# JuliaHealth/Thunderbolt.jl

Hardware: AMD Instinct MI355X
Metric: element-integrations/sec + DoF-updates/sec, 10M-hex Q1 monodomain (higher is better)
Workload: dtype f64

## Files before the change

### thunderbolt.jl_amd/csrc/tb_reaction.hip

```cpp
#include <hip/hip_runtime.h>

#include <cstdlib>
#include <type_traits>

#include "tb_internal.h"
#include "tb_math.hpp"

namespace tb {

struct CellParams {
    double p[48];
};

template <int MODEL> struct CellModel;

template <> struct CellModel<TB_CELL_FHN> {
    static constexpr int NS = 2, PHI = 0;
    static constexpr bool HAS_GATES = false;
    __device__ __forceinline__ static void rhs(const CellParams &P, const double (&u)[NS], double, double (&du)[NS])
    {
        const double a = P.p[0], b = P.p[1], c = P.p[2], d = P.p[3], e = P.p[4], f = P.p[5];
        const double phi = u[0], s = u[1];
        du[0] = f * (phi * (1 - phi) * (phi - a) - s);
        du[1] = e * (b * phi - c * s - d);
    }
};

template <> struct CellModel<TB_CELL_ALIEV_PANFILOV> {
    static constexpr int NS = 2, PHI = 1;
    static constexpr bool HAS_GATES = false;
    __device__ __forceinline__ static void rhs(const CellParams &P, const double (&u)[NS], double, double (&du)[NS])
    {
        const double ct = P.p[0], k = P.p[1], a = P.p[2], e0 = P.p[3], mu1 = P.p[4], mu2 = P.p[5];
        const double phi = u[1], s = u[0];
        const double eps = e0 + s * mu1 / (phi + mu2);
        du[1] = ct * (k * phi * (phi - 1.0) * (phi - a) - phi * s);
        du[0] = ct * eps * (-s - k * phi * (phi - a - 1.0));
    }
};

template <> struct CellModel<TB_CELL_PCG2019> {
    static constexpr int NS = 7, PHI = 0;
    static constexpr bool HAS_GATES = true;
    enum { gNa, Em, km, taum, Eh, kh, dh, tauh0, gK1, Ez, kz, gto, Er, kr, Es, ks, taus, gCaL, Ed, kd, Ef, kf, tauf,
           gKr, Exr, kxr, tauxr, Ey, ky, gKs, Exs, kxs, tauxs, ENa, EK, ECa };
    __device__ __forceinline__ static double sigmoid(double phi, double E, double ik, double sign)
    {
        return rcp_b(1.0 + exp_b(sign * (phi - E) * ik));
    }
    __device__ __forceinline__ static void rhs(const CellParams &P, const double (&u)[NS], double t, double (&du)[NS])
    {
        double rate[NS];
        rhs_rates(P, u, t, du, rate);
    }
    __device__ __forceinline__ static void rhs_rates(const CellParams &P, const double (&u)[NS], double, double (&du)[NS], double (&rate)[NS])
    {
        const double *p = P.p;
        const double phi = u[0], h = u[1], m = u[2], f = u[3], s = u[4], xs = u[5], xr = u[6];
        const double rinf = sigmoid(phi, p[Er], 1.0 / p[kr], -1.0);
        const double dinf = sigmoid(phi, p[Ed], 1.0 / p[kd], -1.0);
        const double zinf = sigmoid(phi, p[Ez], 1.0 / p[kz], 1.0);
        const double yinf = sigmoid(phi, p[Ey], 1.0 / p[ky], 1.0);
        const double I_Na = p[gNa] * m * m * m * h * h * (phi - p[ENa]);
        const double I_K1 = p[gK1] * zinf * (phi - p[EK]);
        const double I_to = p[gto] * rinf * s * (phi - p[EK]);
        const double I_CaL = p[gCaL] * dinf * f * (phi - p[ECa]);
        const double I_Kr = p[gKr] * xr * yinf * (phi - p[EK]);
        const double I_Ks = p[gKs] * xs * (phi - p[EK]);
        du[0] = -(I_Na + I_K1 + I_to + I_CaL + I_Kr + I_Ks);
        const double xh = (phi - p[Eh]) * (1.0 / p[kh]);
        const double eh = exp_b(xh);
        const double hinf = rcp_b(1.0 + eh);
        rate[0] = 0.0; rate[1] = (1.0 + eh) * exp_b(-p[dh] * xh) * (0.5 / p[tauh0]); rate[2] = 1.0 / p[taum]; rate[3] = 1.0 / p[tauf]; rate[4] = 1.0 / p[taus];
        rate[5] = 1.0 / p[tauxs]; rate[6] = 1.0 / p[tauxr];
        du[1] = (hinf - h) * rate[1];
        du[2] = (sigmoid(phi, p[Em], 1.0 / p[km], -1.0) - m) * rate[2];
        du[3] = (sigmoid(phi, p[Ef], 1.0 / p[kf], 1.0) - f) * rate[3];
        du[4] = (sigmoid(phi, p[Es], 1.0 / p[ks], 1.0) - s) * rate[4];
        du[5] = (sigmoid(phi, p[Exs], 1.0 / p[kxs], -1.0) - xs) * rate[5];
        du[6] = (sigmoid(phi, p[Exr], 1.0 / p[kxr], -1.0) - xr) * rate[6];
    }
};

template <> struct CellModel<TB_CELL_FHN_HETEROGENEOUS> {
    static constexpr int NS = 2, PHI = 0;
    static constexpr bool HAS_GATES = false, USES_X = true;
    __device__ __forceinline__ static void rhs_x(const CellParams &P, const double (&u)[NS], const float (&x)[3], double, double (&du)[NS])
    {
        const double a = P.p[0], b = P.p[1], c = P.p[2], d = P.p[3];
        const double e = P.p[4] + P.p[5] * (double)x[0] + P.p[6] * (double)x[1] + P.p[7] * (double)x[2];
        const double phi = u[0], s = u[1];
        du[0] = phi * (1.0 - phi) * (phi - a) - s;
        du[1] = e * (b * phi - c * s - d);
    }
};


template <> struct CellModel<TB_CELL_TT06> {
    static constexpr int NS = 19, PHI = 0;
    __device__ __forceinline__ static double sgm(double e) { return rcp_b(1.0 + e); }
    static constexpr bool HAS_GATES = true;
    __device__ __forceinline__ static void rhs(const CellParams &P, const double (&u)[NS], double t, double (&du)[NS])
    {
        double rate[NS];
        rhs_rates(P, u, t, du, rate);
    }
    __device__ __forceinline__ static void rhs_rates(const CellParams &P, const double (&u)[NS], double, double (&du)[NS], double (&rate)[NS])
    {
#pragma unroll
        for (int k = 0; k < NS; ++k) rate[k] = 0.0;
        const double *p = P.p;
        const double GNa = p[0], GK1 = p[1], GKr = p[2], GKs = p[3], Gto = p[4], GCaL = p[5], GbNa = p[6], GbCa = p[7], GpCa = p[8],
                     GpK = p[9], knak = p[10], knaca = p[11], Ko = p[12], Cao = p[13], Nao = p[14], Vc = p[15], Vsr = p[16], Vss = p[17],
                     Bufc = p[18], Kbufc = p[19], Bufsr = p[20], Kbufsr = p[21], Bufss = p[22], Kbufss = p[23], Vmaxup = p[24], Kup = p[25],
                     Vrel = p[26], k1p = p[27], k2p = p[28], k3 = p[29], k4 = p[30], EC = p[31], maxsr = p[32], minsr = p[33],
                     Vleak = p[34], Vxfer = p[35], Cm = p[36], pKNa = p[37], KmK = p[38], KmNa = p[39], KmNai = p[40], KmCa = p[41],
                     ksat = p[42], nn = p[43], KpCa = p[44], R = p[45], T = p[46], F = p[47];
        const double V = u[0], Cai = u[1], CaSR = u[2], CaSS = u[3], Nai = u[4], Ki = u[5], m = u[6], h = u[7], j = u[8], xr1 = u[9],
                     xr2 = u[10], xs = u[11], r = u[12], s = u[13], d = u[14], f = u[15], f2 = u[16], fCass = u[17], RR = u[18];
        const double RTONF = R * T / F, FoRT = F / (R * T);
        const double Ek = RTONF * (log(Ko) - log_b(Ki)), Ena = RTONF * (log(Nao) - log_b(Nai));
        const double Eks = RTONF * (log(Ko + pKNa * Nao) - log_b(Ki + pKNa * Nai)), Eca = 0.5 * RTONF * (log(Cao) - log_b(Cai));
        const double p5 = exp_b(V * (1.0 / 5.0)), q5 = rcp_b(p5);
        const double p10 = exp_b(V * (1.0 / 10.0)), q10 = rcp_b(p10);
        const double p20 = exp_b(V * (1.0 / 20.0)), q20 = rcp_b(p20);
        const double p7 = exp_b(V * (1.0 / 7.0)), q7 = rcp_b(p7);
        const double q6 = exp_b(-V * (1.0 / 6.0));
        const double w = exp_b(V * FoRT), iw = rcp_b(w);
        const double vk = V - Ek;
        const double Ak1 = 0.1 * sgm(exp_b(0.06 * (vk - 200.0)));
        const double eh = exp_b(-0.5 * vk);
        const double Bk1 = (3.0 * exp_b(0.0002 * (vk + 100.0)) + exp_b(0.1 * (vk - 10.0))) * sgm(eh);
        const double INa = GNa * m * m * m * h * j * (V - Ena);
        const double e2 = w * w * exp_b(-30.0 * FoRT);
        const double ICaL = GCaL * d * f * f2 * fCass * 4.0 * (V - 15.0) * (F * FoRT) * (0.25 * e2 * CaSS - Cao) * rcp_b(e2 - 1.0);
        const double Ito = Gto * r * s * vk;
        const double IKr = GKr * sqrt(Ko * (1.0 / 5.4)) * xr1 * xr2 * vk;
        const double IKs = GKs * xs * xs * (V - Eks);
        const double IK1 = GK1 * (Ak1 * rcp_b(Ak1 + Bk1)) * vk;
        const double en = exp_b(nn * V * FoRT), en1 = en * iw;
        const double INaCa = knaca * (1.0 / (KmNai * KmNai * KmNai + Nao * Nao * Nao)) * (1.0 / (KmCa + Cao)) * rcp_b(1.0 + ksat * en1) *
                             (en * Nai * Nai * Nai * Cao - en1 * Nao * Nao * Nao * Cai * 2.5);
        const double INaK = knak * (Ko / (Ko + KmK)) * (Nai * rcp_b(Nai + KmNa)) * rcp_b(1.0 + 0.1245 * exp_b(-0.1 * V * FoRT) + 0.0353 * iw);
        const double IpCa = GpCa * Cai * rcp_b(KpCa + Cai);
        const double IpK = GpK * sgm(exp_b((25.0 - V) * (1.0 / 5.98))) * vk;
        const double IbNa = GbNa * (V - Ena), IbCa = GbCa * (V - Eca);
        du[0] = -(IKr + IKs + IK1 + Ito + INa + IbNa + ICaL + IbCa + INaK + INaCa + IpCa + IpK);
        const double ecs = EC * rcp_b(CaSR);
        const double kCaSR = maxsr - (maxsr - minsr) * rcp_b(1.0 + ecs * ecs);
        const double k1 = k1p * rcp_b(kCaSR), k2 = k2p * kCaSR;
        du[18] = k4 * (1.0 - RR) - k2 * CaSS * RR;
        const double O = k1 * CaSS * CaSS * RR * rcp_b(k3 + k1 * CaSS * CaSS);
        const double Irel = Vrel * O * (CaSR - CaSS), Ileak = Vleak * (CaSR - Cai);
        const double Iup = Vmaxup * (Cai * Cai) * rcp_b(Cai * Cai + Kup * Kup), Ixfer = Vxfer * (CaSS - Cai);
        const double sc = (Cai + Kbufc) * (Cai + Kbufc), ssr = (CaSR + Kbufsr) * (CaSR + Kbufsr), sss = (CaSS + Kbufss) * (CaSS + Kbufss);
        const double bc = sc * rcp_b(sc + Bufc * Kbufc), bsr = ssr * rcp_b(ssr + Bufsr * Kbufsr), bss = sss * rcp_b(sss + Bufss * Kbufss);
        du[1] = bc * ((Ileak - Iup) * Vsr / Vc + Ixfer - (IbCa + IpCa - 2.0 * INaCa) * Cm / (2.0 * Vc * F));
        du[2] = bsr * (Iup - Irel - Ileak);
        du[3] = bss * (-ICaL * Cm / (2.0 * Vss * F) + Irel * Vsr / Vss - Ixfer * Vc / Vss);
        du[4] = -(INa + IbNa + 3.0 * INaK + 3.0 * INaCa) * Cm / (Vc * F);
        du[5] = -(IK1 + Ito + IKr + IKs - 2.0 * INaK + IpK) * Cm / (Vc * F);
        const double AM = sgm(q5 * 6.14421235332821e-06 );
        const double BM = 0.1 * sgm(p5 * 1096.6331584284585 ) + 0.1 * sgm(exp_b((V - 50.0) * (1.0 / 200.0)));
        const double mr = sgm(exp_b((-56.86 - V) * (1.0 / 9.03)));
        rate[6] = rcp_b(AM * BM);
        du[6] = (mr * mr - m) * rate[6];
        const double hr = sgm(exp_b((V + 71.55) * (1.0 / 7.43)));
        const double hinf = hr * hr;
        double ABH, ABJ;
        if (V >= -40.0) {
            ABH = (0.77 / 0.13) * sgm(exp_b(-(V + 10.66) * (1.0 / 11.1)));
            ABJ = 0.6 * exp_b(0.057 * V) * sgm(q10 * 0.04076220397836621 );
        } else {
            ABH = 0.057 * exp_b(-(V + 80.0) * (1.0 / 6.8)) + 2.7 * exp_b(0.079 * V) + 3.1e5 * exp_b(0.3485 * V);
            ABJ = ((-2.5428e4) * exp_b(0.2444 * V) - 6.948e-6 * exp_b(-0.04391 * V)) * (V + 37.78) * sgm(exp_b(0.311 * (V + 79.23))) +
                  0.02424 * exp_b(-0.01052 * V) * sgm(exp_b(-0.1378 * (V + 40.14)));
        }
        rate[7] = ABH;
        du[7] = (hinf - h) * ABH;
        rate[8] = ABJ;
        du[8] = (hinf - j) * ABJ;
        rate[9] = rcp_b((450.0 * sgm(q10 * 0.011108996538242306 )) * (6.0 * sgm(exp_b((V + 30.0) * (1.0 / 11.5)))));
        du[9] = (sgm(q7 * 0.02437284407327961 ) - xr1) * rate[9];
        rate[10] = rcp_b((3.0 * sgm(q20 * 0.049787068367863944 )) * (1.12 * sgm(p20 * 0.049787068367863944 )));
        du[10] = (sgm(exp_b((V + 88.0) * (1.0 / 24.0))) - xr2) * rate[10];
        rate[11] = rcp_b((1400.0 / sqrt(1.0 + q6 * 2.3009758908928246 )) * sgm(exp_b((V - 35.0) * (1.0 / 15.0))) + 80.0);
        du[11] = (sgm(exp_b((-5.0 - V) * (1.0 / 14.0))) - xs) * rate[11];
        rate[12] = rcp_b(9.5 * exp_b(-(V + 40.0) * (V + 40.0) * (1.0 / 1800.0)) + 0.8);
        du[12] = (sgm(q6 * 28.031624894526125 ) - r) * rate[12];
        rate[13] = rcp_b(85.0 * exp_b(-(V + 45.0) * (V + 45.0) * (1.0 / 320.0)) + 5.0 * sgm(p5 * 0.01831563888873418 ) + 3.0);
        du[13] = (sgm(p5 * 54.598150033144236 ) - s) * rate[13];
        rate[14] = rcp_b((1.4 * sgm(exp_b((-35.0 - V) * (1.0 / 13.0))) + 0.25) * (1.4 * sgm(p5 * 2.718281828459045 )) + sgm(q20 * 12.182493960703473 ));
        du[14] = (sgm(exp_b((-8.0 - V) * (1.0 / 7.5))) - d) * rate[14];
        rate[15] = rcp_b((1102.5 * exp_b(-(V + 27.0) * (V + 27.0) * (1.0 / 225.0)) + 200.0 * sgm(q10 * 3.6692966676192444 ) + 180.0 * sgm(p10 * 20.085536923187668 ) + 20.0));
        du[15] = (sgm(p7 * 17.411708063327644 ) - f) * rate[15];
        rate[16] = rcp_b((600.0 * exp_b(-(V + 25.0) * (V + 25.0) * (1.0 / 170.0)) + 31.0 * sgm(q10 * 12.182493960703473 ) + 16.0 * sgm(p10 * 20.085536923187668 )));
        du[16] = (0.67 * sgm(p7 * 148.4131591025766 ) + 0.33 - f2) * rate[16];
        const double cq = 1.0 + (CaSS * (1.0 / 0.05)) * (CaSS * (1.0 / 0.05));
        const double icq = rcp_b(cq);
        rate[17] = rcp_b(80.0 * icq + 2.0);
        du[17] = (0.6 * icq + 0.4 - fCass) * rate[17];
    }
};


template <> struct CellModel<TB_CELL_ORD11> {
    static constexpr int NS = 41, PHI = 0;
    static constexpr bool HAS_GATES = true;
    __device__ __forceinline__ static double sg(double x) { return rcp_b(1.0 + exp_b(x)); }
    __device__ __forceinline__ static void rhs(const CellParams &P, const double (&u)[NS], double t, double (&du)[NS])
    {
        double rate[NS];
        rhs_rates(P, u, t, du, rate);
    }
    __device__ __forceinline__ static void currents(const CellParams &P, const double (&u)[NS], double (&du)[NS])
    {
        const double *p = P.p;
        const double nao = p[13], cao = p[14], ko = p[15];
        const int celltype = (int)p[16];
        constexpr double R = 8314.0, T = 310.0, F = 96485.0, RTF = R * T / F, FRT = F / (R * T);
        constexpr double L = 0.01, rad = 0.0011, vcell = 1000 * 3.14 * rad * rad * L, Ageo = 2 * 3.14 * rad * rad + 2 * 3.14 * rad * L, Acap = 2 * Ageo;
        constexpr double vmyo = 0.68 * vcell, vnsr = 0.0552 * vcell, vjsr = 0.0048 * vcell, vss = 0.02 * vcell;
        const double v = u[0], nai = u[1], nass = u[2], ki = u[3], kss = u[4], cai = u[5], cass = u[6], cansr = u[7], cajsr = u[8], m = u[9], hf = u[10],
                     hs = u[11], j = u[12], hsp = u[13], jp = u[14], mL = u[15], hL = u[16], hLp = u[17], a = u[18], iF = u[19], iS = u[20],
                     ap = u[21], iFp = u[22], iSp = u[23], d = u[24], ff = u[25], fs = u[26], fcaf = u[27], fcas = u[28], jca = u[29], nca = u[30],
                     ffp = u[31], fcafp = u[32], xrf = u[33], xrs = u[34], xs1 = u[35], xs2 = u[36], xk1 = u[37], Jrelnp = u[38], Jrelp = u[39],
                     CaMKt = u[40];
        constexpr double KmCaMK = 0.15, aCaMK = 0.05, bCaMK = 0.00068, CaMKo = 0.05, KmCaM = 0.0015;
        const double CaMKb = CaMKo * (1.0 - CaMKt) * cass * rcp_b(cass + KmCaM), CaMKa = CaMKb + CaMKt;
        du[40] = aCaMK * CaMKb * (CaMKb + CaMKt) - bCaMK * CaMKt;
        const double fpa = CaMKa * rcp_b(CaMKa + KmCaMK), fnp = 1.0 - fpa;
        const double ENa = RTF * (log(nao) - log(nai)), EK = RTF * (log(ko) - log(ki));
        const double EKs = RTF * (log(ko + 0.01833 * nao) - log(ki + 0.01833 * nai));
        const double vg = fabs(v) < 1e-7 ? 1e-7 : v;
        const double vfrt = vg * FRT, vffrt = vfrt * F;
        constexpr double Ahf = 0.99, Ahs = 1.0 - Ahf;
        const double h = Ahf * hf + Ahs * hs;
        const double hp = Ahf * hf + Ahs * hsp;
        const double INa = 75.0 * p[0] * (v - ENa) * m * m * m * (fnp * h * j + fpa * hp * jp);
        const double INaL = 0.0075 * p[1] * (celltype == 1 ? 0.6 : 1.0) * (v - ENa) * mL * (fnp * hL + fpa * hLp);
        const double AiF = sg((v - 213.6) * (1.0 / 151.2)), AiS = 1.0 - AiF;
        const double i_ = AiF * iF + AiS * iS;
        const double ip = AiF * iFp + AiS * iSp;
        const double Ito = 0.02 * p[2] * (celltype == 0 ? 1.0 : 4.0) * (v - EK) * (fnp * a * i_ + fpa * ap * ip);
        constexpr double Aff = 0.6, Afs = 1.0 - Aff;
        const double f = Aff * ff + Afs * fs;
        const double Afcaf = 0.3 + 0.6 * sg((v - 10.0) * (1.0 / 10.0)), Afcas = 1.0 - Afcaf;
        const double fca = Afcaf * fcaf + Afcas * fcas;
        const double fp = Aff * ffp + Afs * fs;
        const double fcap = Afcaf * fcafp + Afcas * fcas;
        constexpr double Kmn = 0.002, k2n = 1000.0;
        const double km2n = jca;
        const double q1 = 1.0 + Kmn * rcp_b(cass), q2 = q1 * q1;
        const double anca = rcp_b(k2n * rcp_b(km2n) + q2 * q2);
// ... 105 lines not shown
        const double hssp = sg((v + 89.1) * (1.0 / 6.086));
        const double mLss = sg(-(v + 42.85) * (1.0 / 5.264));
        const double hLss = sg((v + 87.61) * (1.0 / 7.488)), hLssp = sg((v + 93.81) * (1.0 / 7.488));
        const double ass = sg(-(v - 14.34) * (1.0 / 14.82));
        const double ta = 1.0515 * rcp_b(sg(-(v - 18.4099) * (1.0 / 29.3814)) * (1.0 / 1.2089) + 3.5 * sg((v + 100.0) * (1.0 / 29.3814)));
        const double iss = sg((v + 43.94) * (1.0 / 5.711));
        const double delta_epi = celltype == 1 ? 1.0 - 0.95 * sg((v + 70.0) * (1.0 / 5.0)) : 1.0;
        const double tiF = (4.562 + rcp_b(0.3933 * exp_b(-(v + 100.0) * (1.0 / 100.0)) + 0.08004 * exp_b((v + 50.0) * (1.0 / 16.59)))) * delta_epi;
        const double tiS = (23.62 + rcp_b(0.001416 * exp_b(-(v + 96.52) * (1.0 / 59.05)) + 1.780e-8 * exp_b((v + 114.1) * (1.0 / 8.079)))) * delta_epi;
        const double assp = sg(-(v - 24.34) * (1.0 / 14.82));
        const double dti_develop = 1.354 + 1.0e-4 * rcp_b(exp_b((v - 167.4) * (1.0 / 15.89)) + exp_b(-(v - 12.23) * (1.0 / 0.2154)));
        const double dti_recover = 1.0 - 0.5 * sg((v + 70.0) * (1.0 / 20.0));
        const double tiFp = dti_develop * dti_recover * tiF, tiSp = dti_develop * dti_recover * tiS;
        const double dss = sg(-(v + 3.940) * (1.0 / 4.230));
        const double td = 0.6 + rcp_b(exp_b(-0.05 * (v + 6.0)) + exp_b(0.09 * (v + 14.0)));
        const double fss = sg((v + 19.58) * (1.0 / 3.696));
        const double e20 = exp_b((v + 20.0) * (1.0 / 10.0));
        const double tff = 7.0 + rcp_b(0.0045 * rcp_b(e20) + 0.0045 * e20);
        const double tfs = 1000.0 + rcp_b(0.000035 * exp_b(-(v + 5.0) * (1.0 / 4.0)) + 0.000035 * exp_b((v + 5.0) * (1.0 / 6.0)));
        const double e4 = exp_b((v - 4.0) * (1.0 / 7.0));
        const double tfcaf = 7.0 + rcp_b(0.04 * rcp_b(e4) + 0.04 * e4);
        const double tfcas = 100.0 + rcp_b(0.00012 * exp_b(-v * (1.0 / 3.0)) + 0.00012 * exp_b(v * (1.0 / 7.0)));
        const double xrss = sg(-(v + 8.337) * (1.0 / 6.789));
        const double txrf = 12.98 + rcp_b(0.3652 * exp_b((v - 31.66) * (1.0 / 3.869)) + 4.123e-5 * exp_b(-(v - 47.78) * (1.0 / 20.38)));
        const double txrs = 1.865 + rcp_b(0.06629 * exp_b((v - 34.70) * (1.0 / 7.355)) + 1.128e-5 * exp_b(-(v - 29.74) * (1.0 / 25.94)));
        const double xs1ss = sg(-(v + 11.60) * (1.0 / 8.932));
        const double txs1 = 817.3 + rcp_b(2.326e-4 * exp_b((v + 48.28) * (1.0 / 17.80)) + 0.001292 * exp_b(-(v + 210.0) * (1.0 / 230.0)));
        const double txs2_r = 0.01 * exp_b((v - 50.0) * (1.0 / 20.0)) + 0.0193 * exp_b(-(v + 66.54) * (1.0 / 31.0));
        const double xk1ss = sg(-(v + 2.5538 * ko + 144.59) / (1.5692 * ko + 3.8115));
        const double txk1_r = (exp_b(-(v + 127.2) * (1.0 / 20.36)) + exp_b((v + 236.8) * (1.0 / 69.33))) * (1.0 / 122.2);
        emit(9, mss, tm_r); emit(10, hss, thf_r); emit(11, hss, ths_r);
        const double rtj = rcp_b(tj);
        emit(12, hss, rtj); emit(13, hssp, ths_r * (1.0 / 3.0)); emit(14, hss, rtj * (1.0 / 1.46));
        emit(15, mLss, tm_r); emit(16, hLss, 1.0 / 200.0); emit(17, hLssp, 1.0 / 600.0);
        const double rta = rcp_b(ta);
        emit(18, ass, rta); emit(19, iss, rcp_b(tiF)); emit(20, iss, rcp_b(tiS)); emit(21, assp, rta); emit(22, iss, rcp_b(tiFp)); emit(23, iss, rcp_b(tiSp));
        emit(24, dss, rcp_b(td)); emit(25, fss, rcp_b(tff)); emit(26, fss, rcp_b(tfs)); emit(27, fss, rcp_b(tfcaf)); emit(28, fss, rcp_b(tfcas));
        emit(29, fss, 1.0 / 75.0); emit(31, fss, rcp_b(tff) * (1.0 / 2.5)); emit(32, fss, rcp_b(tfcaf) * (1.0 / 2.5));
        emit(33, xrss, rcp_b(txrf)); emit(34, xrss, rcp_b(txrs)); emit(35, xs1ss, rcp_b(txs1)); emit(36, xs1ss, txs2_r); emit(37, xk1ss, txk1_r);
    }
    __device__ __forceinline__ static bool is_gate(int k) { return (k >= 9 && k <= 29) || (k >= 31 && k <= 37); }
    __device__ __forceinline__ static void rhs_rates(const CellParams &P, const double (&u)[NS], double, double (&du)[NS], double (&rate)[NS])
    {
#pragma unroll
        for (int k = 0; k < NS; ++k) rate[k] = 0.0;
        currents(P, u, du);
        gates(P, u[0], [&](int k, double inf, double r) { rate[k] = r; du[k] = (inf - u[k]) * r; });
    }
};

template <class M, class = void> struct uses_x : std::false_type {};
template <class M> struct uses_x<M, std::enable_if_t<M::USES_X>> : std::true_type {};

template <class M>
__device__ __forceinline__ void cell_rhs(const CellParams &P, const double (&u)[M::NS], const float (&x)[3], double t, double (&du)[M::NS])
{
    if constexpr (uses_x<M>::value) M::rhs_x(P, u, x, t, du);
    else M::rhs(P, u, t, du);
}

template <int MODEL, int LAYOUT, bool WRITE_DU, class TS = double>
__global__ void __launch_bounds__(256)
k_reaction(CellParams P, TS *__restrict__ u, TS *__restrict__ du_out, int64_t n, double t, double dt, int substeps,
           double threshold, unsigned long long *__restrict__ rmax_key, const float *__restrict__ xs, int sdim, const double *__restrict__ tslot)
{
    if (tslot) t = tslot[0];
    using M = CellModel<MODEL>;
    constexpr int NS = M::NS;
    const int64_t stride = (int64_t)gridDim.x * blockDim.x;
    double rm = -__builtin_huge_val();
    for (int64_t i = (int64_t)blockIdx.x * blockDim.x + threadIdx.x; i < n; i += stride) {
        double ul[NS], dul[NS];
#pragma unroll
        for (int j = 0; j < NS; ++j) ul[j] = LAYOUT == TB_LAYOUT_SOA ? u[i + j * n] : u[i * NS + j];
        float xp[3] = {0.0f, 0.0f, 0.0f};
        if constexpr (uses_x<M>::value) {
            if (xs) for (int d = 0; d < sdim; ++d) xp[d] = xs[i * sdim + d];
        }
        cell_rhs<M>(P, ul, xp, t, dul);
        if (substeps <= 1 || fabs(dul[M::PHI]) < threshold) {
#pragma unroll
            for (int j = 0; j < NS; ++j) ul[j] += dt * dul[j];
        } else {
            const double dts = dt / substeps;
#pragma unroll
            for (int j = 0; j < NS; ++j) ul[j] += dts * dul[j];
            for (int s = 2; s <= substeps; ++s) {
                cell_rhs<M>(P, ul, xp, t + (s - 1) * dts, dul);
#pragma unroll
                for (int j = 0; j < NS; ++j) ul[j] += dts * dul[j];
            }
        }
#pragma unroll
        for (int j = 0; j < NS; ++j) {
            const int64_t k = LAYOUT == TB_LAYOUT_SOA ? i + j * n : i * NS + j;
            u[k] = (TS)ul[j];
            if (WRITE_DU) du_out[k] = (TS)dul[j];
        }
        rm = fmax(rm, dul[M::PHI]);
    }
    if (rmax_key) {
#pragma unroll
        for (int o = 32; o > 0; o >>= 1) rm = fmax(rm, __shfl_xor(rm, o, 64));
        if ((threadIdx.x & 63) == 0) {
            const unsigned long long b = (unsigned long long)__double_as_longlong(rm);
            atomicMax(rmax_key, (b >> 63) ? ~b : (b | 0x8000000000000000ull));
        }
    }
}

__device__ __forceinline__ double expm1_b(double z)
{
    if (fabs(z) < 0.3) {
        double q = 1.6059043836821613e-10;
        const double c[11] = {2.08767569878681e-09, 2.505210838544172e-08, 2.755731922398589e-07, 2.7557319223985893e-06, 2.48015873015873e-05,
                              0.0001984126984126984, 0.001388888888888889, 0.008333333333333333, 0.041666666666666664, 0.16666666666666666, 0.5};
#pragma unroll
        for (int i = 0; i < 11; ++i) q = fma(q, z, c[i]);
        q = fma(q, z, 1.0);
        return q * z;
    }
    return exp_b(z) - 1.0;
}

template <int MODEL, int LAYOUT>
__global__ void __launch_bounds__(256)
k_reaction_rl(CellParams P, double *__restrict__ u, int64_t n, double t, double dt, const double *__restrict__ tslot)
{
    if (tslot) t = tslot[0];
    using M = CellModel<MODEL>;
    constexpr int NS = M::NS;
    const int64_t stride = (int64_t)gridDim.x * blockDim.x;
    for (int64_t i = (int64_t)blockIdx.x * blockDim.x + threadIdx.x; i < n; i += stride) {
        double ul[NS], dul[NS], rate[NS];
#pragma unroll
        for (int j = 0; j < NS; ++j) ul[j] = LAYOUT == TB_LAYOUT_SOA ? u[i + j * n] : u[i * NS + j];
        M::rhs_rates(P, ul, t, dul, rate);
#pragma unroll
        for (int j = 0; j < NS; ++j) {
            const double h = rate[j] != 0.0 ? -expm1_b(-dt * rate[j]) * rcp_b(rate[j]) : dt;
            const int64_t k = LAYOUT == TB_LAYOUT_SOA ? i + j * n : i * NS + j;
            u[k] = ul[j] + h * dul[j];
        }
    }
}

int launch_reaction_rl(tb_device *dev, int model, const double *params, int n_params, double *d_u, int64_t n, int layout, double t, double dt)
{
    if (model != TB_CELL_TT06 && model != TB_CELL_PCG2019 && model != TB_CELL_ORD11) {
        set_error("Rush–Larsen step: cell model %d has no gate decomposition (TB_CELL_TT06, TB_CELL_PCG2019 and TB_CELL_ORD11 have)", model);
        return TB_ERR_UNSUPPORTED;
    }
    CellParams P{};
    for (int i = 0; i < n_params && i < 48; ++i) P.p[i] = params[i];
    int64_t nb = (n + 255) / 256;
    const int64_t cap = (int64_t)dev->n_cu * 16;
    if (nb > cap) nb = (nb + (nb + cap - 1) / cap - 1) / ((nb + cap - 1) / cap);
    if (n == 0) return TB_OK;
    const double *ts = dev->capturing ? (dev->tslot_used = true, dev->d_tslot) : nullptr;
#define TB_RL(MODEL) do { if (layout == TB_LAYOUT_SOA) hipLaunchKernelGGL((k_reaction_rl<MODEL, TB_LAYOUT_SOA>), dim3((unsigned)nb), dim3(256), 0, dev->stream, P, d_u, n, t, dt, ts); \
                          else hipLaunchKernelGGL((k_reaction_rl<MODEL, TB_LAYOUT_AOS>), dim3((unsigned)nb), dim3(256), 0, dev->stream, P, d_u, n, t, dt, ts); } while (0)
    if (model == TB_CELL_TT06) TB_RL(TB_CELL_TT06); else if (model == TB_CELL_ORD11) TB_RL(TB_CELL_ORD11); else TB_RL(TB_CELL_PCG2019);
#undef TB_RL
    TB_HIP(hipGetLastError());
    return TB_OK;
}

template <int MODEL, class TS = double>
static int run(tb_device *dev, const CellParams &P, TS *u, TS *du, int64_t n, int layout, double t, double dt, int substeps,
               double thr, unsigned long long *rmax_key, const float *xs, int sdim)
{
    const int bs = 256;
    auto launch = [&](auto kern) -> int {
        static struct { const void *f; int occ; } seen[8];
        int occ = 0;
        for (auto &e : seen) if (e.f == (const void *)kern) occ = e.occ;
        if (!occ) {
            if (hipOccupancyMaxActiveBlocksPerMultiprocessor(&occ, kern, bs, 0) != hipSuccess || occ < 1) occ = 1;
            for (auto &e : seen) if (!e.f) { e.f = (const void *)kern; e.occ = occ; break; }
        }
        int64_t nb = (n + bs - 1) / bs;
        static const int per_cu_env = tune_env("TB_REACTION_BLOCKS_PER_CU") ? atoi(tune_env("TB_REACTION_BLOCKS_PER_CU")) : -1;
        const int64_t resident = (int64_t)dev->n_cu * occ;
        const int64_t cap = per_cu_env > 0 ? (int64_t)dev->n_cu * per_cu_env : per_cu_env == 0 ? nb : (nb <= 12 * resident ? resident : 2 * resident);
        if (nb > cap) nb = (nb + (nb + cap - 1) / cap - 1) / ((nb + cap - 1) / cap);
        hipLaunchKernelGGL(kern, dim3((unsigned)nb), dim3(bs), 0, dev->stream, P, u, du, n, t, dt, substeps, thr, rmax_key, xs, sdim,
                           dev->capturing ? (dev->tslot_used = true, (const double *)dev->d_tslot) : (const double *)nullptr);
        return TB_OK;
    };
    if (layout == TB_LAYOUT_SOA) { if (du) launch(k_reaction<MODEL, TB_LAYOUT_SOA, true, TS>); else launch(k_reaction<MODEL, TB_LAYOUT_SOA, false, TS>); }
    else { if (du) launch(k_reaction<MODEL, TB_LAYOUT_AOS, true, TS>); else launch(k_reaction<MODEL, TB_LAYOUT_AOS, false, TS>); }
    TB_HIP(hipGetLastError());
    return TB_OK;
}

int launch_reaction_f32(tb_device *dev, int model, const double *params, int n_params, float *d_u, float *d_du, int64_t n_points,
                        int layout, double t, double dt, int substeps, double thr, const float *d_x, int sdim)
{
    CellParams P{};
    for (int i = 0; i < n_params && i < 48; ++i) P.p[i] = params[i];
    switch (model) {
    case TB_CELL_FHN: return run<TB_CELL_FHN, float>(dev, P, d_u, d_du, n_points, layout, t, dt, substeps, thr, nullptr, d_x, sdim);
    case TB_CELL_ALIEV_PANFILOV: return run<TB_CELL_ALIEV_PANFILOV, float>(dev, P, d_u, d_du, n_points, layout, t, dt, substeps, thr, nullptr, d_x, sdim);
    case TB_CELL_PCG2019: return run<TB_CELL_PCG2019, float>(dev, P, d_u, d_du, n_points, layout, t, dt, substeps, thr, nullptr, d_x, sdim);
    case TB_CELL_TT06: return run<TB_CELL_TT06, float>(dev, P, d_u, d_du, n_points, layout, t, dt, substeps, thr, nullptr, d_x, sdim);
    case TB_CELL_FHN_HETEROGENEOUS: return run<TB_CELL_FHN_HETEROGENEOUS, float>(dev, P, d_u, d_du, n_points, layout, t, dt, substeps, thr, nullptr, d_x, sdim);
    case TB_CELL_ORD11: return run<TB_CELL_ORD11, float>(dev, P, d_u, d_du, n_points, layout, t, dt, substeps, thr, nullptr, d_x, sdim);
    default: set_error("unknown cell model %d", model); return TB_ERR_BAD_ARG;
    }
}

int launch_reaction(tb_device *dev, int model, const double *params, int n_params, double *d_u, double *d_du, int64_t n_points,
                    int layout, double t, double dt, int substeps, double thr, double *rmax, const float *d_x, int sdim)
{
    CellParams P{};
    for (int i = 0; i < n_params && i < 48; ++i) P.p[i] = params[i];
    unsigned long long *key = nullptr;
    if (rmax) {
        TB_NO_CAPTURE(dev);
        key = (unsigned long long *)&dev->d_status->cell;
        TB_HIP(hipMemsetAsync(key, 0, sizeof *key, dev->stream));
    }
    int rc = TB_ERR_BAD_ARG;
    switch (model) {
    case TB_CELL_FHN: rc = run<TB_CELL_FHN>(dev, P, d_u, d_du, n_points, layout, t, dt, substeps, thr, key, d_x, sdim); break;
// ... 17 lines not shown
```

Before: 11.38 billion.

## Fold TT06 constants on host and algebraically simplify gate rate expressions

Precomputes the TT06 parameter-only subexpressions (log of external concentrations, volume ratios, NaCa and NaK prefactors and similar) on the host into a folded parameter struct passed to the kernel. The per-cell math is rewritten to share exponentials (p5 and p10 derived from p20 by squaring) and to merge nested reciprocals of sigmoids into single divisions, cutting transcendental and rcp counts. Loop-invariant n is also hidden behind an opaque inline asm so that strided SoA address computation stays scalar. The rewritten expressions can differ slightly in rounding from the original formulas.

Result: faster. 11.54 billion, median of 6 (+1.4%).

```diff
diff --git a/thunderbolt.jl_amd/csrc/tb_reaction.hip b/thunderbolt.jl_amd/csrc/tb_reaction.hip
--- a/thunderbolt.jl_amd/csrc/tb_reaction.hip
+++ b/thunderbolt.jl_amd/csrc/tb_reaction.hip
@@ -1,5 +1,6 @@
 #include <hip/hip_runtime.h>
 
+#include <cmath>
 #include <cstdlib>
 #include <type_traits>
 
@@ -96,19 +97,22 @@
 };
 
 
+struct TT06Folded {
+    enum { GNa, GK1, GKr , GKs, Gto, GCaL , GbNa, GbCa, GpCa, GpK, NaK , KmNa,
+           NaCa1 , NaCa2 , ksat, Cao, KpCa,
+           RTONF, Ek0 , Ena0 , Eks0 , Eca0 , pKNa, FoRT,
+           E30 , nnFoRT, EC2 , maxsr, dsr , k1p, k2p, k3, k4, Vrel, Vleak, Vmaxup, Kup2, Vxfer,
+           Kbufc, BKc , Kbufsr, BKsr, Kbufss, BKss, VsrVc , CaVc , CaVss ,
+           VsrVss, VcVss, NaVc , NF };
+    double c[NF];
+    __host__ __device__ double operator[](int k) const { return c[k]; }
+};
+
 template <> struct CellModel<TB_CELL_TT06> {
     static constexpr int NS = 19, PHI = 0;
-    __device__ __forceinline__ static double sgm(double e) { return rcp_b(1.0 + e); }
-    static constexpr bool HAS_GATES = true;
-    __device__ __forceinline__ static void rhs(const CellParams &P, const double (&u)[NS], double t, double (&du)[NS])
-    {
-        double rate[NS];
-        rhs_rates(P, u, t, du, rate);
-    }
-    __device__ __forceinline__ static void rhs_rates(const CellParams &P, const double (&u)[NS], double, double (&du)[NS], double (&rate)[NS])
-    {
-#pragma unroll
-        for (int k = 0; k < NS; ++k) rate[k] = 0.0;
+    using Params = TT06Folded;
+    static TT06Folded fold(const CellParams &P)
+    {
         const double *p = P.p;
         const double GNa = p[0], GK1 = p[1], GKr = p[2], GKs = p[3], Gto = p[4], GCaL = p[5], GbNa = p[6], GbCa = p[7], GpCa = p[8],
                      GpK = p[9], knak = p[10], knaca = p[11], Ko = p[12], Cao = p[13], Nao = p[14], Vc = p[15], Vsr = p[16], Vss = p[17],
@@ -116,54 +120,88 @@
                      Vrel = p[26], k1p = p[27], k2p = p[28], k3 = p[29], k4 = p[30], EC = p[31], maxsr = p[32], minsr = p[33],
                      Vleak = p[34], Vxfer = p[35], Cm = p[36], pKNa = p[37], KmK = p[38], KmNa = p[39], KmNai = p[40], KmCa = p[41],
                      ksat = p[42], nn = p[43], KpCa = p[44], R = p[45], T = p[46], F = p[47];
+        const double RTONF = R * T / F, FoRT = F / (R * T);
+        const double naca = knaca * (1.0 / (KmNai * KmNai * KmNai + Nao * Nao * Nao)) * (1.0 / (KmCa + Cao));
+        TT06Folded f{};
+        double *c = f.c;
+        c[TT06Folded::GNa] = GNa; c[TT06Folded::GK1] = GK1; c[TT06Folded::GKr] = GKr * std::sqrt(Ko * (1.0 / 5.4)); c[TT06Folded::GKs] = GKs;
+        c[TT06Folded::Gto] = Gto; c[TT06Folded::GCaL] = GCaL * 4.0 * (F * FoRT); c[TT06Folded::GbNa] = GbNa; c[TT06Folded::GbCa] = GbCa;
+        c[TT06Folded::GpCa] = GpCa; c[TT06Folded::GpK] = GpK; c[TT06Folded::NaK] = knak * (Ko / (Ko + KmK)); c[TT06Folded::KmNa] = KmNa;
+        c[TT06Folded::NaCa1] = naca * Cao; c[TT06Folded::NaCa2] = naca * (Nao * Nao * Nao * 2.5); c[TT06Folded::ksat] = ksat;
+        c[TT06Folded::Cao] = Cao; c[TT06Folded::KpCa] = KpCa;
+        c[TT06Folded::RTONF] = RTONF; c[TT06Folded::Ek0] = RTONF * std::log(Ko); c[TT06Folded::Ena0] = RTONF * std::log(Nao);
+        c[TT06Folded::Eks0] = RTONF * std::log(Ko + pKNa * Nao); c[TT06Folded::Eca0] = 0.5 * RTONF * std::log(Cao); c[TT06Folded::pKNa] = pKNa;
+        c[TT06Folded::FoRT] = FoRT; c[TT06Folded::E30] = std::exp(-30.0 * FoRT); c[TT06Folded::nnFoRT] = nn * FoRT;
+        c[TT06Folded::EC2] = EC * EC; c[TT06Folded::maxsr] = maxsr; c[TT06Folded::dsr] = maxsr - minsr; c[TT06Folded::k1p] = k1p;
+        c[TT06Folded::k2p] = k2p; c[TT06Folded::k3] = k3; c[TT06Folded::k4] = k4; c[TT06Folded::Vrel] = Vrel; c[TT06Folded::Vleak] = Vleak;
+        c[TT06Folded::Vmaxup] = Vmaxup; c[TT06Folded::Kup2] = Kup * Kup; c[TT06Folded::Vxfer] = Vxfer;
+        c[TT06Folded::Kbufc] = Kbufc; c[TT06Folded::BKc] = Bufc * Kbufc; c[TT06Folded::Kbufsr] = Kbufsr; c[TT06Folded::BKsr] = Bufsr * Kbufsr;
+        c[TT06Folded::Kbufss] = Kbufss; c[TT06Folded::BKss] = Bufss * Kbufss;
+        c[TT06Folded::VsrVc] = Vsr / Vc; c[TT06Folded::CaVc] = Cm / (2.0 * Vc * F); c[TT06Folded::CaVss] = Cm / (2.0 * Vss * F);
+        c[TT06Folded::VsrVss] = Vsr / Vss; c[TT06Folded::VcVss] = Vc / Vss; c[TT06Folded::NaVc] = Cm / (Vc * F);
+        return f;
+    }
+    __device__ __forceinline__ static double sgm(double e) { return rcp_b(1.0 + e); }
+    static constexpr bool HAS_GATES = true;
+    __device__ __forceinline__ static void rhs(const TT06Folded &c, const double (&u)[NS], double t, double (&du)[NS])
+    {
+        double rate[NS];
+        rhs_rates(c, u, t, du, rate);
+    }
+    __device__ __forceinline__ static void rhs_rates(const TT06Folded &c, const double (&u)[NS], double, double (&du)[NS], double (&rate)[NS])
+    {
+        using C = TT06Folded;
+#pragma unroll
+        for (int k = 0; k < NS; ++k) rate[k] = 0.0;
         const double V = u[0], Cai = u[1], CaSR = u[2], CaSS = u[3], Nai = u[4], Ki = u[5], m = u[6], h = u[7], j = u[8], xr1 = u[9],
                      xr2 = u[10], xs = u[11], r = u[12], s = u[13], d = u[14], f = u[15], f2 = u[16], fCass = u[17], RR = u[18];
-        const double RTONF = R * T / F, FoRT = F / (R * T);
-        const double Ek = RTONF * (log(Ko) - log_b(Ki)), Ena = RTONF * (log(Nao) - log_b(Nai));
-        const double Eks = RTONF * (log(Ko + pKNa * Nao) - log_b(Ki + pKNa * Nai)), Eca = 0.5 * RTONF * (log(Cao) - log_b(Cai));
-        const double p5 = exp_b(V * (1.0 / 5.0)), q5 = rcp_b(p5);
-        const double p10 = exp_b(V * (1.0 / 10.0)), q10 = rcp_b(p10);
-        const double p20 = exp_b(V * (1.0 / 20.0)), q20 = rcp_b(p20);
+        const double RTONF = c[C::RTONF], FoRT = c[C::FoRT];
+        const double Ek = fma(-RTONF, log_b(Ki), c[C::Ek0]), Ena = fma(-RTONF, log_b(Nai), c[C::Ena0]);
+        const double Eks = fma(-RTONF, log_b(Ki + c[C::pKNa] * Nai), c[C::Eks0]), Eca = fma(-0.5 * RTONF, log_b(Cai), c[C::Eca0]);
+        const double p20 = exp_b(V * (1.0 / 20.0)), p10 = p20 * p20, p5 = p10 * p10;
+        const double q20 = rcp_b(p20), q10 = q20 * q20, q5 = q10 * q10;
         const double p7 = exp_b(V * (1.0 / 7.0)), q7 = rcp_b(p7);
         const double q6 = exp_b(-V * (1.0 / 6.0));
         const double w = exp_b(V * FoRT), iw = rcp_b(w);
         const double vk = V - Ek;
-        const double Ak1 = 0.1 * sgm(exp_b(0.06 * (vk - 200.0)));
-        const double eh = exp_b(-0.5 * vk);
-        const double Bk1 = (3.0 * exp_b(0.0002 * (vk + 100.0)) + exp_b(0.1 * (vk - 10.0))) * sgm(eh);
-        const double INa = GNa * m * m * m * h * j * (V - Ena);
-        const double e2 = w * w * exp_b(-30.0 * FoRT);
-        const double ICaL = GCaL * d * f * f2 * fCass * 4.0 * (V - 15.0) * (F * FoRT) * (0.25 * e2 * CaSS - Cao) * rcp_b(e2 - 1.0);
-        const double Ito = Gto * r * s * vk;
-        const double IKr = GKr * sqrt(Ko * (1.0 / 5.4)) * xr1 * xr2 * vk;
-        const double IKs = GKs * xs * xs * (V - Eks);
-        const double IK1 = GK1 * (Ak1 * rcp_b(Ak1 + Bk1)) * vk;
-        const double en = exp_b(nn * V * FoRT), en1 = en * iw;
-        const double INaCa = knaca * (1.0 / (KmNai * KmNai * KmNai + Nao * Nao * Nao)) * (1.0 / (KmCa + Cao)) * rcp_b(1.0 + ksat * en1) *
-                             (en * Nai * Nai * Nai * Cao - en1 * Nao * Nao * Nao * Cai * 2.5);
-        const double INaK = knak * (Ko / (Ko + KmK)) * (Nai * rcp_b(Nai + KmNa)) * rcp_b(1.0 + 0.1245 * exp_b(-0.1 * V * FoRT) + 0.0353 * iw);
-        const double IpCa = GpCa * Cai * rcp_b(KpCa + Cai);
-        const double IpK = GpK * sgm(exp_b((25.0 - V) * (1.0 / 5.98))) * vk;
-        const double IbNa = GbNa * (V - Ena), IbCa = GbCa * (V - Eca);
+        const double a1 = exp_b(0.06 * (vk - 200.0)), g = exp_b(0.1 * vk), g2 = g * g, g5 = g2 * g2 * g;
+        const double Bk = 3.0 * exp_b(0.0002 * (vk + 100.0)) + g * 0.36787944117144233 ;
+        const double nk1 = 0.1 * (g5 + 1.0);
+        const double xk1 = nk1 * rcp_b(fma(Bk * (1.0 + a1), g5, nk1));
+        const double INa = c[C::GNa] * m * m * m * h * j * (V - Ena);
+        const double e2 = w * w * c[C::E30];
+        const double ICaL = c[C::GCaL] * d * f * f2 * fCass * (V - 15.0) * (0.25 * e2 * CaSS - c[C::Cao]) * rcp_b(e2 - 1.0);
+        const double Ito = c[C::Gto] * r * s * vk;
+        const double IKr = c[C::GKr] * xr1 * xr2 * vk;
+        const double IKs = c[C::GKs] * xs * xs * (V - Eks);
+        const double IK1 = c[C::GK1] * xk1 * vk;
+        const double en = exp_b(c[C::nnFoRT] * V), en1 = en * iw;
+        const double INaCa = rcp_b(fma(c[C::ksat], en1, 1.0)) * (en * Nai * Nai * Nai * c[C::NaCa1] - en1 * Cai * c[C::NaCa2]);
+        const double INaK = c[C::NaK] * Nai * rcp_b((Nai + c[C::KmNa]) * (1.0 + 0.1245 * exp_b(-0.1 * V * FoRT) + 0.0353 * iw));
+        const double IpCa = c[C::GpCa] * Cai * rcp_b(c[C::KpCa] + Cai);
+        const double IpK = c[C::GpK] * sgm(exp_b((25.0 - V) * (1.0 / 5.98))) * vk;
+        const double IbNa = c[C::GbNa] * (V - Ena), IbCa = c[C::GbCa] * (V - Eca);
         du[0] = -(IKr + IKs + IK1 + Ito + INa + IbNa + ICaL + IbCa + INaK + INaCa + IpCa + IpK);
-        const double ecs = EC * rcp_b(CaSR);
-        const double kCaSR = maxsr - (maxsr - minsr) * rcp_b(1.0 + ecs * ecs);
-        const double k1 = k1p * rcp_b(kCaSR), k2 = k2p * kCaSR;
-        du[18] = k4 * (1.0 - RR) - k2 * CaSS * RR;
-        const double O = k1 * CaSS * CaSS * RR * rcp_b(k3 + k1 * CaSS * CaSS);
-        const double Irel = Vrel * O * (CaSR - CaSS), Ileak = Vleak * (CaSR - Cai);
-        const double Iup = Vmaxup * (Cai * Cai) * rcp_b(Cai * Cai + Kup * Kup), Ixfer = Vxfer * (CaSS - Cai);
-        const double sc = (Cai + Kbufc) * (Cai + Kbufc), ssr = (CaSR + Kbufsr) * (CaSR + Kbufsr), sss = (CaSS + Kbufss) * (CaSS + Kbufss);
-        const double bc = sc * rcp_b(sc + Bufc * Kbufc), bsr = ssr * rcp_b(ssr + Bufsr * Kbufsr), bss = sss * rcp_b(sss + Bufss * Kbufss);
-        du[1] = bc * ((Ileak - Iup) * Vsr / Vc + Ixfer - (IbCa + IpCa - 2.0 * INaCa) * Cm / (2.0 * Vc * F));
+        const double sr2 = CaSR * CaSR;
+        const double kCaSR = c[C::maxsr] - c[C::dsr] * sr2 * rcp_b(sr2 + c[C::EC2]);
+        const double k2 = c[C::k2p] * kCaSR;
+        du[18] = c[C::k4] * (1.0 - RR) - k2 * CaSS * RR;
+        const double kss = c[C::k1p] * CaSS * CaSS;
+        const double O = kss * RR * rcp_b(fma(c[C::k3], kCaSR, kss));
+        const double Irel = c[C::Vrel] * O * (CaSR - CaSS), Ileak = c[C::Vleak] * (CaSR - Cai);
+        const double Iup = c[C::Vmaxup] * (Cai * Cai) * rcp_b(Cai * Cai + c[C::Kup2]), Ixfer = c[C::Vxfer] * (CaSS - Cai);
+        const double sc = (Cai + c[C::Kbufc]) * (Cai + c[C::Kbufc]), ssr = (CaSR + c[C::Kbufsr]) * (CaSR + c[C::Kbufsr]),
+                     sss = (CaSS + c[C::Kbufss]) * (CaSS + c[C::Kbufss]);
+        const double bc = sc * rcp_b(sc + c[C::BKc]), bsr = ssr * rcp_b(ssr + c[C::BKsr]), bss = sss * rcp_b(sss + c[C::BKss]);
+        du[1] = bc * ((Ileak - Iup) * c[C::VsrVc] + Ixfer - (IbCa + IpCa - 2.0 * INaCa) * c[C::CaVc]);
         du[2] = bsr * (Iup - Irel - Ileak);
-        du[3] = bss * (-ICaL * Cm / (2.0 * Vss * F) + Irel * Vsr / Vss - Ixfer * Vc / Vss);
-        du[4] = -(INa + IbNa + 3.0 * INaK + 3.0 * INaCa) * Cm / (Vc * F);
-        du[5] = -(IK1 + Ito + IKr + IKs - 2.0 * INaK + IpK) * Cm / (Vc * F);
-        const double AM = sgm(q5 * 6.14421235332821e-06 );
-        const double BM = 0.1 * sgm(p5 * 1096.6331584284585 ) + 0.1 * sgm(exp_b((V - 50.0) * (1.0 / 200.0)));
+        du[3] = bss * (-ICaL * c[C::CaVss] + Irel * c[C::VsrVss] - Ixfer * c[C::VcVss]);
+        du[4] = -(INa + IbNa + 3.0 * INaK + 3.0 * INaCa) * c[C::NaVc];
+        du[5] = -(IK1 + Ito + IKr + IKs - 2.0 * INaK + IpK) * c[C::NaVc];
+        const double mA = q5 * 6.14421235332821e-06 , mB = p5 * 1096.6331584284585 ;
+        const double mC = exp_b((V - 50.0) * (1.0 / 200.0));
         const double mr = sgm(exp_b((-56.86 - V) * (1.0 / 9.03)));
-        rate[6] = rcp_b(AM * BM);
+        rate[6] = (1.0 + mA) * (1.0 + mB) * (1.0 + mC) * rcp_b(0.1 * (2.0 + mB + mC));
         du[6] = (mr * mr - m) * rate[6];
         const double hr = sgm(exp_b((V + 71.55) * (1.0 / 7.43)));
         const double hinf = hr * hr;
@@ -173,33 +211,41 @@
             ABJ = 0.6 * exp_b(0.057 * V) * sgm(q10 * 0.04076220397836621 );
         } else {
             ABH = 0.057 * exp_b(-(V + 80.0) * (1.0 / 6.8)) + 2.7 * exp_b(0.079 * V) + 3.1e5 * exp_b(0.3485 * V);
-            ABJ = ((-2.5428e4) * exp_b(0.2444 * V) - 6.948e-6 * exp_b(-0.04391 * V)) * (V + 37.78) * sgm(exp_b(0.311 * (V + 79.23))) +
-                  0.02424 * exp_b(-0.01052 * V) * sgm(exp_b(-0.1378 * (V + 40.14)));
+            const double X = ((-2.5428e4) * exp_b(0.2444 * V) - 6.948e-6 * exp_b(-0.04391 * V)) * (V + 37.78), Y = 0.02424 * exp_b(-0.01052 * V);
+            const double b1 = 1.0 + exp_b(0.311 * (V + 79.23)), b2 = 1.0 + exp_b(-0.1378 * (V + 40.14));
+            ABJ = (X * b2 + Y * b1) * rcp_b(b1 * b2);
         }
         rate[7] = ABH;
         du[7] = (hinf - h) * ABH;
         rate[8] = ABJ;
         du[8] = (hinf - j) * ABJ;
-        rate[9] = rcp_b((450.0 * sgm(q10 * 0.011108996538242306 )) * (6.0 * sgm(exp_b((V + 30.0) * (1.0 / 11.5)))));
+        rate[9] = (1.0 + q10 * 0.011108996538242306 ) * (1.0 + exp_b((V + 30.0) * (1.0 / 11.5))) * (1.0 / 2700.0);
         du[9] = (sgm(q7 * 0.02437284407327961 ) - xr1) * rate[9];
-        rate[10] = rcp_b((3.0 * sgm(q20 * 0.049787068367863944 )) * (1.12 * sgm(p20 * 0.049787068367863944 )));
+        rate[10] = (1.0 + q20 * 0.049787068367863944 ) * (1.0 + p20 * 0.049787068367863944 ) * (1.0 / (3.0 * 1.12));
         du[10] = (sgm(exp_b((V + 88.0) * (1.0 / 24.0))) - xr2) * rate[10];
-        rate[11] = rcp_b((1400.0 / sqrt(1.0 + q6 * 2.3009758908928246 )) * sgm(exp_b((V - 35.0) * (1.0 / 15.0))) + 80.0);
+        const double zs = sqrt(1.0 + q6 * 2.3009758908928246 ) * (1.0 + exp_b((V - 35.0) * (1.0 / 15.0)));
+        rate[11] = zs * rcp_b(fma(80.0, zs, 1400.0));
         du[11] = (sgm(exp_b((-5.0 - V) * (1.0 / 14.0))) - xs) * rate[11];
         rate[12] = rcp_b(9.5 * exp_b(-(V + 40.0) * (V + 40.0) * (1.0 / 1800.0)) + 0.8);
         du[12] = (sgm(q6 * 28.031624894526125 ) - r) * rate[12];
-        rate[13] = rcp_b(85.0 * exp_b(-(V + 45.0) * (V + 45.0) * (1.0 / 320.0)) + 5.0 * sgm(p5 * 0.01831563888873418 ) + 3.0);
+        const double sA = 1.0 + p5 * 0.01831563888873418 ;
+        rate[13] = sA * rcp_b(fma(85.0 * exp_b(-(V + 45.0) * (V + 45.0) * (1.0 / 320.0)) + 3.0, sA, 5.0));
         du[13] = (sgm(p5 * 54.598150033144236 ) - s) * rate[13];
-        rate[14] = rcp_b((1.4 * sgm(exp_b((-35.0 - V) * (1.0 / 13.0))) + 0.25) * (1.4 * sgm(p5 * 2.718281828459045 )) + sgm(q20 * 12.182493960703473 ));
+        const double da = 1.0 + exp_b((-35.0 - V) * (1.0 / 13.0)), db = 1.0 + p5 * 2.718281828459045 ,
+                     dc = 1.0 + q20 * 12.182493960703473 ;
+        const double dab = da * db;
+        rate[14] = dab * dc * rcp_b(fma(1.4 * (0.25 * da + 1.4), dc, dab));
         du[14] = (sgm(exp_b((-8.0 - V) * (1.0 / 7.5))) - d) * rate[14];
-        rate[15] = rcp_b((1102.5 * exp_b(-(V + 27.0) * (V + 27.0) * (1.0 / 225.0)) + 200.0 * sgm(q10 * 3.6692966676192444 ) + 180.0 * sgm(p10 * 20.085536923187668 ) + 20.0));
+        const double fA = 1.0 + q10 * 3.6692966676192444 , fB = 1.0 + p10 * 20.085536923187668 , fAB = fA * fB;
+        rate[15] = fAB * rcp_b(fma(1102.5 * exp_b(-(V + 27.0) * (V + 27.0) * (1.0 / 225.0)) + 20.0, fAB, 200.0 * fB + 180.0 * fA));
         du[15] = (sgm(p7 * 17.411708063327644 ) - f) * rate[15];
-        rate[16] = rcp_b((600.0 * exp_b(-(V + 25.0) * (V + 25.0) * (1.0 / 170.0)) + 31.0 * sgm(q10 * 12.182493960703473 ) + 16.0 * sgm(p10 * 20.085536923187668 )));
+        const double gA = 1.0 + q10 * 12.182493960703473 , gAB = gA * fB;
+        rate[16] = gAB * rcp_b(fma(600.0 * exp_b(-(V + 25.0) * (V + 25.0) * (1.0 / 170.0)), gAB, 31.0 * fB + 16.0 * gA));
         du[16] = (0.67 * sgm(p7 * 148.4131591025766 ) + 0.33 - f2) * rate[16];
         const double cq = 1.0 + (CaSS * (1.0 / 0.05)) * (CaSS * (1.0 / 0.05));
-        const double icq = rcp_b(cq);
-        rate[17] = rcp_b(80.0 * icq + 2.0);
-        du[17] = (0.6 * icq + 0.4 - fCass) * rate[17];
+        const double icq = rcp_b(fma(2.0, cq, 80.0));
+        rate[17] = cq * icq;
+        du[17] = fma(0.4 - fCass, cq, 0.6) * icq;
     }
 };
 
@@ -411,8 +457,23 @@
 template <class M, class = void> struct uses_x : std::false_type {};
 template <class M> struct uses_x<M, std::enable_if_t<M::USES_X>> : std::true_type {};
 
+template <class M, class = void> struct params_of {
+    using type = CellParams;
+    static const CellParams &fold(const CellParams &P) { return P; }
+};
+template <class M> struct params_of<M, std::void_t<typename M::Params>> {
+    using type = typename M::Params;
+    static type fold(const CellParams &P) { return M::fold(P); }
+};
+
+__device__ __forceinline__ int64_t opaque_uniform(int64_t v)
+{
+    asm volatile("" : "+s"(v));
+    return v;
+}
+
 template <class M>
-__device__ __forceinline__ void cell_rhs(const CellParams &P, const double (&u)[M::NS], const float (&x)[3], double t, double (&du)[M::NS])
+__device__ __forceinline__ void cell_rhs(const typename params_of<M>::type &P, const double (&u)[M::NS], const float (&x)[3], double t, double (&du)[M::NS])
 {
     if constexpr (uses_x<M>::value) M::rhs_x(P, u, x, t, du);
     else M::rhs(P, u, t, du);
@@ -420,7 +481,7 @@
 
 template <int MODEL, int LAYOUT, bool WRITE_DU, class TS = double>
 __global__ void __launch_bounds__(256)
-k_reaction(CellParams P, TS *__restrict__ u, TS *__restrict__ du_out, int64_t n, double t, double dt, int substeps,
+k_reaction(typename params_of<CellModel<MODEL>>::type P, TS *__restrict__ u, TS *__restrict__ du_out, int64_t n, double t, double dt, int substeps,
            double threshold, unsigned long long *__restrict__ rmax_key, const float *__restrict__ xs, int sdim, const double *__restrict__ tslot)
 {
     if (tslot) t = tslot[0];
@@ -430,8 +491,9 @@
     double rm = -__builtin_huge_val();
     for (int64_t i = (int64_t)blockIdx.x * blockDim.x + threadIdx.x; i < n; i += stride) {
         double ul[NS], dul[NS];
-#pragma unroll
-        for (int j = 0; j < NS; ++j) ul[j] = LAYOUT == TB_LAYOUT_SOA ? u[i + j * n] : u[i * NS + j];
+        const int64_t nl = opaque_uniform(n);
+#pragma unroll
+        for (int j = 0; j < NS; ++j) ul[j] = LAYOUT == TB_LAYOUT_SOA ? u[i + j * nl] : u[i * NS + j];
         float xp[3] = {0.0f, 0.0f, 0.0f};
         if constexpr (uses_x<M>::value) {
             if (xs) for (int d = 0; d < sdim; ++d) xp[d] = xs[i * sdim + d];
@@ -450,9 +512,10 @@
                 for (int j = 0; j < NS; ++j) ul[j] += dts * dul[j];
             }
         }
+        const int64_t ns = opaque_uniform(n);
 #pragma unroll
         for (int j = 0; j < NS; ++j) {
-            const int64_t k = LAYOUT == TB_LAYOUT_SOA ? i + j * n : i * NS + j;
+            const int64_t k = LAYOUT == TB_LAYOUT_SOA ? i + j * ns : i * NS + j;
             u[k] = (TS)ul[j];
             if (WRITE_DU) du_out[k] = (TS)dul[j];
         }
@@ -484,7 +547,7 @@
 
 template <int MODEL, int LAYOUT>
 __global__ void __launch_bounds__(256)
-k_reaction_rl(CellParams P, double *__restrict__ u, int64_t n, double t, double dt, const double *__restrict__ tslot)
+k_reaction_rl(typename params_of<CellModel<MODEL>>::type P, double *__restrict__ u, int64_t n, double t, double dt, const double *__restrict__ tslot)
 {
     if (tslot) t = tslot[0];
     using M = CellModel<MODEL>;
@@ -492,13 +555,15 @@
     const int64_t stride = (int64_t)gridDim.x * blockDim.x;
     for (int64_t i = (int64_t)blockIdx.x * blockDim.x + threadIdx.x; i < n; i += stride) {
         double ul[NS], dul[NS], rate[NS];
-#pragma unroll
-        for (int j = 0; j < NS; ++j) ul[j] = LAYOUT == TB_LAYOUT_SOA ? u[i + j * n] : u[i * NS + j];
+        const int64_t nl = opaque_uniform(n);
+#pragma unroll
+        for (int j = 0; j < NS; ++j) ul[j] = LAYOUT == TB_LAYOUT_SOA ? u[i + j * nl] : u[i * NS + j];
         M::rhs_rates(P, ul, t, dul, rate);
+        const int64_t ns = opaque_uniform(n);
 #pragma unroll
         for (int j = 0; j < NS; ++j) {
             const double h = rate[j] != 0.0 ? -expm1_b(-dt * rate[j]) * rcp_b(rate[j]) : dt;
-            const int64_t k = LAYOUT == TB_LAYOUT_SOA ? i + j * n : i * NS + j;
+            const int64_t k = LAYOUT == TB_LAYOUT_SOA ? i + j * ns : i * NS + j;
             u[k] = ul[j] + h * dul[j];
         }
     }
@@ -517,8 +582,9 @@
     if (nb > cap) nb = (nb + (nb + cap - 1) / cap - 1) / ((nb + cap - 1) / cap);
     if (n == 0) return TB_OK;
     const double *ts = dev->capturing ? (dev->tslot_used = true, dev->d_tslot) : nullptr;
-#define TB_RL(MODEL) do { if (layout == TB_LAYOUT_SOA) hipLaunchKernelGGL((k_reaction_rl<MODEL, TB_LAYOUT_SOA>), dim3((unsigned)nb), dim3(256), 0, dev->stream, P, d_u, n, t, dt, ts); \
-                          else hipLaunchKernelGGL((k_reaction_rl<MODEL, TB_LAYOUT_AOS>), dim3((unsigned)nb), dim3(256), 0, dev->stream, P, d_u, n, t, dt, ts); } while (0)
+#define TB_RL(MODEL) do { const auto PF = params_of<CellModel<MODEL>>::fold(P); \
+                          if (layout == TB_LAYOUT_SOA) hipLaunchKernelGGL((k_reaction_rl<MODEL, TB_LAYOUT_SOA>), dim3((unsigned)nb), dim3(256), 0, dev->stream, PF, d_u, n, t, dt, ts); \
+                          else hipLaunchKernelGGL((k_reaction_rl<MODEL, TB_LAYOUT_AOS>), dim3((unsigned)nb), dim3(256), 0, dev->stream, PF, d_u, n, t, dt, ts); } while (0)
     if (model == TB_CELL_TT06) TB_RL(TB_CELL_TT06); else if (model == TB_CELL_ORD11) TB_RL(TB_CELL_ORD11); else TB_RL(TB_CELL_PCG2019);
 #undef TB_RL
     TB_HIP(hipGetLastError());
@@ -526,10 +592,11 @@
 }
 
 template <int MODEL, class TS = double>
-static int run(tb_device *dev, const CellParams &P, TS *u, TS *du, int64_t n, int layout, double t, double dt, int substeps,
+static int run(tb_device *dev, const CellParams &P0, TS *u, TS *du, int64_t n, int layout, double t, double dt, int substeps,
                double thr, unsigned long long *rmax_key, const float *xs, int sdim)
 {
     const int bs = 256;
+    const auto P = params_of<CellModel<MODEL>>::fold(P0);
     auto launch = [&](auto kern) -> int {
         static struct { const void *f; int occ; } seen[8];
         int occ = 0;
```
